# probabilists/azula

Hardware: AMD Instinct MI355X
Metric: images/sec (whole node), DDIM-64 256x256 UNet (higher is better)
Workload: dtype f32 (f16x2 split: 2 half pieces per operand, 3 partial products, f32 accumulate)

## Files before the change

### azula_amd/_lib.py

```python

from __future__ import annotations

import ctypes as C
import functools
import os
import threading

import torch

_HERE = os.path.dirname(os.path.abspath(__file__))
LIB_PATH = os.environ.get("AZULA_AMD_LIB") or os.path.join(_HERE, "csrc", "libazula_amd.so")

c_f32p = C.c_void_p
c_stream = C.c_void_p


class AzStepCoef(C.Structure):
    _fields_ = [
        ("c_in", C.c_float),
        ("c_skip", C.c_float),
        ("c_out", C.c_float),
        ("c_time", C.c_float),
        ("alpha_t", C.c_float),
        ("alpha_s", C.c_float),
# ... 279 lines not shown
        ("qk_heads", C.c_int32),
        ("qk_tokens", C.c_int32),
        ("qk_rmsnorm", C.c_int32),
        ("qk_eps", C.c_float),
        ("qk_reserved", C.c_int32),
        ("qk_q_weight", c_f32p),
        ("qk_k_weight", c_f32p),
        ("qk_rope_cos", c_f32p),
        ("qk_rope_sin", c_f32p),
        ("depth_wrap", C.c_int32),
        ("dst_dtype", C.c_int32),
        ("w_scale", C.c_float),
        ("reserved1", C.c_int32),
        ("in_absmax0", c_f32p),
        ("in_absmax1", c_f32p),
    ]


class AzAttnArgs(C.Structure):
    _fields_ = [
        ("q", c_f32p),
        ("k", c_f32p),
        ("v", c_f32p),
        ("out", c_f32p),
        ("batch", C.c_int32),
        ("heads", C.c_int32),
        ("tokens", C.c_int32),
        ("head_dim", C.c_int32),
        ("q_bstride", C.c_int64),
        ("q_tstride", C.c_int64),
# ... 125 lines not shown
    "az_conv2d_winograd_f32": [C.POINTER(AzConvArgs), c_stream],
    "az_conv2d_winograd_suggest_splitk": [i64, i32, i32, i32, i32],
    "az_winograd_pack_filter_f32": [vp, vp, i32, i32, i32, i32, i32, i32, c_stream],
    "az_conv2d_winograd_x3_f32": [C.POINTER(AzConvArgs), c_stream],
    "az_winograd_pack_filter_x3_f32": [vp, vp, i32, i32, i32, i32, i32, i32, c_stream],
    "az_winograd_x3_choose_block": [i32, i32, i32, i32, vp, vp, vp, vp],
    "az_winograd_x3_block_geometry": [i32, i32, i32, i32, i32, i32, i32, vp, vp],
    "az_winograd_x3_structured_mask": [C.POINTER(AzConvArgs), vp, vp],
    "az_conv2d_f16x2_f32": [C.POINTER(AzConvArgs), c_stream],
    "az_conv2d_winograd_f16x2_f32": [C.POINTER(AzConvArgs), c_stream],
    "az_pack_conv_weight_f16x2_f32": [vp, vp, i32, i32, i32, i32, i32, i32, i32, f32, c_stream],
    "az_winograd_pack_filter_f16x2_f32": [vp, vp, i32, i32, i32, i32, i32, i32, f32, c_stream],
    "az_f16x2_weight_scale": [f32, i32],
    "az_absmax_f32": [vp, vp, i64, c_stream],
    "az_absmax_from_moments_f32": [vp, vp, i64, c_stream],
    "az_conv2d_winograd4_f32": [C.POINTER(AzConvArgs), c_stream],
    "az_conv2d_winograd4_suggest_splitk": [i64, i32, i32, i32, i32],
    "az_winograd4_pack_filter_f32": [vp, vp, i32, i32, i32, i32, i32, i32, c_stream],
    "az_pack_conv_weight_f32": [vp, vp, i32, i32, i32, i32, i32, i32, i32, c_stream],
    "az_attention_f32": [C.POINTER(AzAttnArgs), c_stream],
    "az_attention_x3_f32": [C.POINTER(AzAttnArgs), c_stream],
    "az_attention_f16x2_f32": [C.POINTER(AzAttnArgs), c_stream],
    "az_attention_bf16_f32": [C.POINTER(AzAttnArgs), c_stream],
    "az_attention_f16_f32": [C.POINTER(AzAttnArgs), c_stream],
    "az_qk_prep_f32": [vp, vp, vp, vp, i64, i64, i32, i32, i64, i64, i64, i64, i64, i64, i32, i32, f32, vp, vp, c_stream],
    "az_qk_prep_w_f32": [vp, vp, vp, vp, i64, i64, i32, i32, i64, i64, i64, i64, i64, i64, i32, i32, f32, vp, vp, vp, vp, c_stream],
    "az_qk_prep_bwd_f32": [vp, vp, vp, vp, vp, vp, i64, i64, i32, i32, i64, i64, i64, i64, i64, i64, i64, i64, i64, i32, i32, f32, vp, vp,
                           c_stream],
    "az_qk_prep_bwd_w_f32": [vp, vp, vp, vp, vp, vp, i64, i64, i32, i32, i64, i64, i64, i64, i64, i64, i64, i64, i64, i32, i32, f32, vp,
                             vp, vp, vp, c_stream],
# ... 86 lines not shown
```

### azula_amd/csrc/conv.hip

```cpp
#include "conv_shared.h"
#include <cstdio>
#include <cstdlib>
#include <type_traits>

namespace {

constexpr int BM = 128;
constexpr int BN = 128;
constexpr int BK = 32;
constexpr int LDSS = 36;
constexpr int TILE_F = (BM + BN) * LDSS;

#include "igemm_kloop.inc"
struct ConvP {
  AzConvArgs a;
  int npix;
  int cin_s;
  int nkc0;
  int nkc1;
  int nk;
  int kps;
  int tiles_m;
  int tiles_n;
  int asm_loop;
// ... 1423 lines not shown
    }
    epilogue_store<IO>(a, n, co, v);
  }
}

template <int IO = 0>
__global__ __launch_bounds__(256) void conv_splitk_reduce_stats_kernel(ConvP p, int cpix) {
  __shared__ float sh[3 * 256];
  const AzConvArgs& a = p.a;
  const int Q = a.cout_s / 4;
  const int hw = a.hout * a.wout;
  const int b = blockIdx.y, chunk = blockIdx.x;
  const int tid = threadIdx.x;
  const int slots = Q >= 256 ? 1 : 256 / Q;
  const int p0 = chunk * cpix, p1 = min(hw, p0 + cpix);
  for (int q0 = 0; q0 < Q; q0 += 256) {
    const int q = q0 + (Q >= 256 ? tid : tid % Q);
    const int slot = Q >= 256 ? 0 : tid / Q;
    float cnt = 0.f, pivot = 0.f, s1 = 0.f, s2 = 0.f;
    if (q < Q && slot < slots) {
      for (int px = p0 + slot; px < p1; px += slots) {
        const int n = b * hw + px;
        float4 v = make_float4(0.f, 0.f, 0.f, 0.f);
#pragma unroll 4
        for (int z = 0; z < a.splitk; ++z) {
          const float4 w = ld4(a.workspace + ((int64_t)z * p.npix + n) * a.cout_s + q * 4);
          v.x += w.x;
          v.y += w.y;
          v.z += w.z;
          v.w += w.w;
// ... 26 lines not shown
          if (nb > 0.f) {
            const float nn = cnt + nb, d = mb - mean;
            mean = mean + d * (nb / nn);
            m2 = (m2 + vb) + d * d * (cnt * nb / nn);
            cnt = nn;
          }
        }
      }
    }
    if (slot == 0 && q < Q) {
      float* out = a.gn_quads + (((int64_t)b * a.gn_chunks + chunk) * Q + q) * 4;
      out[0] = cnt;
      out[1] = mean;
      out[2] = m2;
      out[3] = 0.f;
    }
  }
}

constexpr int WT = 64;
constexpr int WC = 64;
constexpr int WK = 8;
constexpr int WU_STAGE = 16 * WC * WK;
constexpr int WV_STAGE = 16 * WT * WK;
constexpr int W_STAGE = WU_STAGE + WV_STAGE;
constexpr int W_OT = 4 * WC + 4;
constexpr int W_LDS_BYTES = (2 * WT * W_OT + 3 * WT + 384) * 4;



__device__ __forceinline__ int wswz(int row, int half) { return row * WK + 4 * (half ^ ((row >> 3) & 1)); }
// ... 792 lines not shown
    const int grid = az_stream_grid((int64_t)cp.npix * (a.cout_s / 4), 256);
    if (io == 1) hipLaunchKernelGGL(conv_splitk_reduce_kernel<1>, dim3(grid), dim3(256), 0, st, cp);
    else if (io == 2) hipLaunchKernelGGL(conv_splitk_reduce_kernel<2>, dim3(grid), dim3(256), 0, st, cp);
    else hipLaunchKernelGGL(conv_splitk_reduce_kernel<0>, dim3(grid), dim3(256), 0, st, cp);
  }
  return az_launch_status();
}

static int conv2d_direct(const AzConvArgs* a, az_stream_t stream, int half );

int az_conv2d_f32(const AzConvArgs* a, az_stream_t stream) { return conv2d_direct(a, stream, 0); }

int az_conv2d_stem_f32(const AzConvArgs* a, az_stream_t stream) {
  AZ_REQUIRE(a && a->src0 && a->weight && a->dst, AZ_E_NULL);
  AZ_REQUIRE(a->ksize == 3 && a->stride == 1 && a->pad == 1 && !a->aniso && !a->src1 && a->c1s == 0 && a->up0 == 0 && !a->gate &&
                 !a->res && !a->dst_nchw && !a->in_affine && a->depth == 0 && a->splitk <= 1 && (a->act == 0 || a->act == 1),
             AZ_E_UNSUPPORTED);
  AZ_REQUIRE(a->c0s >= 1 && a->c0s <= 4 && a->cout_s > 0 && a->cout_s % 4 == 0 && a->batch > 0 && a->hin > 0 && a->win > 0 &&
                 a->hout == a->hin && a->wout == a->win && a->h0 == a->hin && a->w0 == a->win,
             AZ_E_SHAPE);
  AZ_REQUIRE((int64_t)a->batch * a->hin * a->win * a->cout_s < (1ll << 40), AZ_E_SHAPE);
  AZ_REQUIRE(AZ_ALIGNED16(a->weight) && AZ_ALIGNED16(a->bias) && AZ_ALIGNED16(a->dst) && AZ_ALIGNED16(a->gn_quads), AZ_E_ALIGN);
  const int tiles_h = (a->hin + ST_TH - 1) / ST_TH, tiles_w = (a->win + ST_TW - 1) / ST_TW;
  const int tiles_img = tiles_h * tiles_w;
  AZ_REQUIRE((int64_t)a->batch * tiles_img < (1ll << 31), AZ_E_SHAPE);
  if (a->gn_quads) AZ_REQUIRE(a->gn_chunks == tiles_img, AZ_E_SHAPE);
  ConvP p{};
  p.a = *a;
  const dim3 grid((unsigned)(a->batch * tiles_img));
  hipStream_t st = az_s(stream);
  switch (a->c0s) {
// ... 11 lines not shown
int az_conv2d_f16x2_f32(const AzConvArgs* a, az_stream_t stream) { return conv2d_direct(a, stream, 4); }

static bool conv_pow2(float v) {
  int e;
  return v > 0.f && v < 3.0e38f && frexpf(v, &e) == 0.5f;
}

static void launch_igemm_half(const ConvP& p, bool f16, bool srch, dim3 grid, hipStream_t st) {
  if (f16 && srch) hipLaunchKernelGGL((conv_igemm_half_kernel<true, true>), grid, dim3(256), 0, st, p);
  else if (f16) hipLaunchKernelGGL((conv_igemm_half_kernel<true, false>), grid, dim3(256), 0, st, p);
  else if (srch) hipLaunchKernelGGL((conv_igemm_half_kernel<false, true>), grid, dim3(256), 0, st, p);
  else hipLaunchKernelGGL((conv_igemm_half_kernel<false, false>), grid, dim3(256), 0, st, p);
}

static int conv2d_direct(const AzConvArgs* a, az_stream_t stream, int half) {
  AZ_REQUIRE(!a || !a->in_affine, AZ_E_UNSUPPORTED);
  if (a && a->depth != 0)
    AZ_REQUIRE(a->depth > 0 && a->batch % a->depth == 0 && a->depth_shift > -a->depth && a->depth_shift < a->depth &&
                   a->cout_s != 4 && (!a->gate || a->gate_bstride == 0) && (a->depth_wrap == 0 || a->depth_wrap == 1),
               AZ_E_UNSUPPORTED);
  AZ_REQUIRE(a && a->src0 && a->weight && a->dst, AZ_E_NULL);
  AZ_REQUIRE(a->batch > 0 && a->hin > 0 && a->win > 0 && a->hout > 0 && a->wout > 0, AZ_E_SHAPE);
  if (a->depth > 0) {
    const int64_t span = (int64_t)BN / ((int64_t)a->hout * a->wout) + 2 + a->depth;
    AZ_REQUIRE(span * a->h0 * a->w0 * a->c0s * 4 < (1ll << 31) && span * a->h1 * a->w1 * a->c1s * 4 < (1ll << 31), AZ_E_SHAPE);
  }
  AZ_REQUIRE(a->c0s > 0 && a->c0s % 4 == 0 && a->c1s % 4 == 0 && a->cout_s > 0 && a->cout_s % 4 == 0, AZ_E_SHAPE);
  AZ_REQUIRE((a->c1s == 0) == (a->src1 == nullptr), AZ_E_SHAPE);
  AZ_REQUIRE((a->src_dtype == 0 || a->src_dtype == 1) && (a->dst_dtype == 0 || a->dst_dtype == 1), AZ_E_SHAPE);
  AZ_REQUIRE((a->src_dtype == 0 && a->dst_dtype == 0) || half == 1 || half == 2, AZ_E_UNSUPPORTED);
  if (a->src_dtype) AZ_REQUIRE(a->c0s % 8 == 0 && a->c1s % 8 == 0, AZ_E_SHAPE);
// ... 316 lines not shown
      p.tblocks = a->batch * x3_rect_blocks_per_image(p.tiles_h, p.tiles_w, rw, rh);
      wino_order(p, 16);
    }
  }
  p.ups = x3_launch_mask(p.a);
  if (h2) AZ_REQUIRE(conv_pow2(a->w_scale), AZ_E_SHAPE);
  p.out_scale = h2 ? 1.f / a->w_scale : 1.f;
  if (h2) AZ_REQUIRE(AZ_ALIGNED16(a->in_absmax0) && AZ_ALIGNED16(a->in_absmax1) && (a->in_absmax0 || !a->in_absmax1), AZ_E_ALIGN);
  hipStream_t st = az_s(stream);
  int rc = azi_winograd_x3_launch(p, (unsigned)splitk, st, h2);
  if (rc != AZ_OK) return rc;
  if (splitk > 1) {
    ConvP cp;
    cp.a = p.a;
    cp.a.gn_quads = a->gn_quads;
    cp.npix = p.npix;
    rc = launch_splitk_reduce(cp, st);
  }
  return rc;
}

static void wino_order(WinoP& p, int wk) {
  int env_gt = 0, env_gc = 0;
  if (const char* e = az_ab_env("AZ_WINO_RECT")) sscanf(e, "%d,%d", &env_gt, &env_gc);
  int gt = env_gt > 0 ? env_gt : 8, gc = env_gt > 0 ? (env_gc > 0 ? env_gc : p.cblocks) : (wk == 16 ? 2 : 4);
  while (gc > 1 && p.cblocks % gc) gc >>= 1;
  if (env_gt <= 0) gt = 32 / gc;
  while (gt > 1 && p.tblocks % gt) gt >>= 1;
  if (p.cblocks % gc || p.tblocks % gt) gt = 1, gc = p.cblocks;
  p.gt = gt, p.gc = gc;
// ... 32 lines not shown
                 AZ_ALIGNED16(a->gate) && AZ_ALIGNED16(a->res) && AZ_ALIGNED16(a->workspace),
             AZ_E_ALIGN);
  if (!a->dst_nchw) AZ_REQUIRE(AZ_ALIGNED16(a->dst), AZ_E_ALIGN);
  if (a->dst_nchw) AZ_REQUIRE(a->dst_c > 0 && a->dst_c <= a->cout_s, AZ_E_SHAPE);
  if (a->gate) AZ_REQUIRE(a->gate_bstride % 4 == 0, AZ_E_ALIGN);
  if (a->res && a->res_up) AZ_REQUIRE(((a->hout + 1) >> 1) <= a->hres && ((a->wout + 1) >> 1) <= a->wres, AZ_E_SHAPE);
  AZ_REQUIRE(a->splitk >= 1 && (a->splitk == 1 || a->workspace), AZ_E_SHAPE);
  const int64_t npix64 = (int64_t)a->batch * a->hout * a->wout;
  AZ_REQUIRE(npix64 < (1ll << 31), AZ_E_SHAPE);
  if (a->gn_quads && a->splitk == 1) {
    const int64_t tiles_img = (int64_t)((a->hout + 1) / 2) * ((a->wout + 1) / 2);
    AZ_REQUIRE(!a->dst_nchw && a->cout_s % WC == 0 && tiles_img % WT == 0 && a->hout % 2 == 0 &&
                   a->wout % 2 == 0 && a->gn_chunks == tiles_img / WT,
               AZ_E_UNSUPPORTED);
  }

  p.a = *a;
  p.npix = (int)npix64;
  p.tiles_h = (a->hout + 1) / 2;
  p.tiles_w = (a->wout + 1) / 2;
  p.ntiles = a->batch * p.tiles_h * p.tiles_w;
  p.nkc0 = (a->c0s + wk - 1) / wk;
  p.nkc1 = (a->c1s + wk - 1) / wk;
  p.nk = p.nkc0 + p.nkc1;
  {
    const int64_t tiles_img = (int64_t)p.tiles_h * p.tiles_w;
    const int64_t span = (WT + tiles_img - 1) / tiles_img + 1;
    AZ_REQUIRE(span * a->h0 * a->w0 * a->c0s * 4 < (1ll << 31), AZ_E_SHAPE);
    AZ_REQUIRE(span * a->h1 * a->w1 * a->c1s * 4 < (1ll << 31), AZ_E_SHAPE);
  }
  splitk = a->splitk;
  if (splitk > p.nk) splitk = p.nk;
  p.kps = (p.nk + splitk - 1) / splitk;
  splitk = (p.nk + p.kps - 1) / p.kps;
  p.a.splitk = splitk;
  AZ_REQUIRE(!a->gn_quads || (a->splitk == 1) == (splitk == 1), AZ_E_UNSUPPORTED);
  if (splitk > 1) p.a.gn_quads = nullptr;
  p.cblocks = (a->cout_s + WC - 1) / WC;
  p.tblocks = (p.ntiles + WT - 1) / WT;
  p.rect_w = WT, p.rect_h = 1;
  p.ups = 0;
  wino_order(p, wk);
  AZ_REQUIRE((int64_t)p.nk * p.cblocks * ustage_bytes <= (1ll << 31), AZ_E_SHAPE);
  return AZ_OK;
}

int az_conv2d_winograd_suggest_splitk(int64_t batch, int32_t hout, int32_t wout, int32_t cout_s, int32_t cin_s) {
  const int64_t tiles = batch * ((hout + 1) / 2) * ((wout + 1) / 2);
  const int64_t blocks = ((tiles + WT - 1) / WT) * ((cout_s + WC - 1) / WC);
  const int64_t nk = (cin_s + WK - 1) / WK;
  int64_t want = (256 + blocks - 1) / blocks;
  int64_t maxs = nk / 8;
// ... 1 lines not shown
  if (want > maxs) want = maxs;
  if (want > 16) want = 16;
  if (blocks >= 192) want = 1;
  return (int)(want < 1 ? 1 : want);
}

int az_conv2d_winograd4_f32(const AzConvArgs* a, az_stream_t stream) {
  AZ_REQUIRE(a && a->src0 && a->weight && a->dst, AZ_E_NULL);
  AZ_REQUIRE(a->ksize == 3 && a->stride == 1 && a->pad == 1 && !a->aniso && a->src_dtype == 0 && a->dst_dtype == 0, AZ_E_UNSUPPORTED);
  AZ_REQUIRE(a->batch > 0 && a->hin > 0 && a->win > 0 && a->hout == a->hin && a->wout == a->win, AZ_E_SHAPE);
  AZ_REQUIRE(a->c0s > 0 && a->c0s % 4 == 0 && a->c1s % 4 == 0 && a->cout_s > 0 && a->cout_s % 4 == 0, AZ_E_SHAPE);
  AZ_REQUIRE((a->c1s == 0) == (a->src1 == nullptr), AZ_E_SHAPE);
  AZ_REQUIRE((a->act >= 0 && a->act <= 4) || a->act == 6, AZ_E_UNSUPPORTED);
  if (a->act == 6) AZ_REQUIRE(a->res && !a->gate && !a->dst_nchw && !a->gn_quads, AZ_E_UNSUPPORTED);
  if (a->act == 4) AZ_REQUIRE(!a->gate && !a->res && !a->dst_nchw && !a->gn_quads && a->cout_s % 8 == 0, AZ_E_UNSUPPORTED);
  AZ_REQUIRE(!a->in_affine && a->depth == 0, AZ_E_UNSUPPORTED);
  AZ_REQUIRE(!a->aniso || (a->up0_w >= 0 && a->up0_w <= 4 && a->up1_w >= 0 && a->up1_w <= 4), AZ_E_SHAPE);
  AZ_REQUIRE(a->up0 >= 0 && a->up0 <= 4 && ((a->hin + (1 << a->up0) - 1) >> a->up0) <= a->h0 &&
                 ((a->win + (1 << az_upw(a, a->up0, a->up0_w)) - 1) >> az_upw(a, a->up0, a->up0_w)) <= a->w0,
             AZ_E_SHAPE);
  if (a->src1)
    AZ_REQUIRE(a->up1 >= 0 && a->up1 <= 4 && ((a->hin + (1 << a->up1) - 1) >> a->up1) <= a->h1 &&
                 ((a->win + (1 << az_upw(a, a->up1, a->up1_w)) - 1) >> az_upw(a, a->up1, a->up1_w)) <= a->w1,
             AZ_E_SHAPE);
  AZ_REQUIRE(AZ_ALIGNED16(a->src0) && AZ_ALIGNED16(a->src1) && AZ_ALIGNED16(a->weight) && AZ_ALIGNED16(a->bias) &&
                 AZ_ALIGNED16(a->gate) && AZ_ALIGNED16(a->res) && AZ_ALIGNED16(a->workspace),
             AZ_E_ALIGN);
  if (!a->dst_nchw) AZ_REQUIRE(AZ_ALIGNED16(a->dst), AZ_E_ALIGN);
  if (a->dst_nchw) AZ_REQUIRE(a->dst_c > 0 && a->dst_c <= a->cout_s, AZ_E_SHAPE);
  if (a->gate) AZ_REQUIRE(a->gate_bstride % 4 == 0, AZ_E_ALIGN);
  if (a->res && a->res_up) AZ_REQUIRE(((a->hout + 1) >> 1) <= a->hres && ((a->wout + 1) >> 1) <= a->wres, AZ_E_SHAPE);
// ... 63 lines not shown
```

### azula_amd/csrc/conv_shared.h

```cpp
#pragma once

#include "common.h"

namespace {

typedef float f32x16 __attribute__((ext_vector_type(16)));

__device__ __forceinline__ float4 ld4(const float* p) { return *reinterpret_cast<const float4*>(p); }


typedef unsigned int u32x4 __attribute__((ext_vector_type(4)));

__device__ __forceinline__ float4 buf_ld4(__amdgpu_buffer_rsrc_t rsrc, unsigned voff, unsigned soff) {
  const u32x4 v = __builtin_amdgcn_raw_buffer_load_b128(rsrc, (int)voff, (int)soff, 0);
  return __builtin_bit_cast(float4, v);
}

typedef float f32x2 __attribute__((ext_vector_type(2)));
typedef unsigned int u32x2 __attribute__((ext_vector_type(2)));

__device__ __forceinline__ f32x2 buf_ld2(__amdgpu_buffer_rsrc_t rsrc, unsigned voff, unsigned soff) {
  const u32x2 v = __builtin_amdgcn_raw_buffer_load_b64(rsrc, (int)voff, (int)soff, 0);
  return __builtin_bit_cast(f32x2, v);
}
// ... 11 lines not shown

__device__ __forceinline__ int az_depth_plane(const AzConvArgs& a, int b, bool& ok) {
  ok = true;
  if (a.depth <= 0) return b;
  const int bd = b % a.depth;
  int sb = bd + a.depth_shift;
  if (a.depth_wrap) sb = sb < 0 ? sb + a.depth : (sb >= a.depth ? sb - a.depth : sb);
  else ok = (unsigned)sb < (unsigned)a.depth;
  return b - bd + sb;
}
__device__ __forceinline__ int az_depth_base(const AzConvArgs& a, int b_first) {
  if (a.depth <= 0) return b_first;
  if (a.depth_wrap) return b_first - b_first % a.depth;
  const int s = b_first + a.depth_shift;
  return s > 0 ? s : 0;
}

static inline int az_upw(const AzConvArgs* a, int up, int up_w) { return a->aniso ? up_w : up; }

__device__ __forceinline__ int64_t epilogue_res_index(const AzConvArgs& a, int n, int b) {
  const int rem = n - b * (a.hout * a.wout);
  if (a.res_up) {
    const int oh = rem / a.wout, ow = rem - oh * a.wout;
    return ((int64_t)b * a.hres + (oh >> 1)) * a.wres + (ow >> 1);
  }
  return a.res_bcast ? rem : n;
}

template <int IO = 0>
__device__ __forceinline__ void epilogue_fetch(const AzConvArgs& a, int n, int b, int co, float4& gate, float4& res) {
// ... 339 lines not shown
```

### azula_amd/csrc/norm.hip

```cpp
#include "common.h"

namespace {

struct Moments {
  float n, mean, m2;
};

__device__ __forceinline__ Moments combine(Moments a, Moments b) {
  if (b.n == 0.f) return a;
  if (a.n == 0.f) return b;
  Moments r;
  r.n = a.n + b.n;
  const float d = b.mean - a.mean;
  const float f = b.n / r.n;
  r.mean = a.mean + d * f;
  r.m2 = a.m2 + b.m2 + d * d * a.n * f;
  return r;
}

template <int IO = 0>
__global__ __launch_bounds__(256) void gn_stats_vec_kernel(float* __restrict__ partials,
                                                           const float* __restrict__ x,
                                                           const float* __restrict__ x1, int c0s, int64_t HW, int C,
                                                           int cs, int groups, int nchunks, int qs) {
// ... 537 lines not shown
}

__global__ __launch_bounds__(256) void absmax_moments_kernel(float* __restrict__ slots, const float4* __restrict__ partials, int64_t count) {
  __shared__ float sh[4];
  float m = 0.f;
  for (int64_t i = (int64_t)blockIdx.x * 256 + threadIdx.x; i < count; i += (int64_t)gridDim.x * 256) {
    const float4 q = partials[i];
    if (q.x > 0.f) m = fmaxf(m, fabsf(q.y) + sqrtf(fmaxf(q.z, 0.f)));
  }
  m = az_wave_max(m);
  if ((threadIdx.x & 63) == 0) sh[threadIdx.x >> 6] = m;
  __syncthreads();
  if (threadIdx.x == 0) slots[blockIdx.x] = fmaxf(fmaxf(sh[0], sh[1]), fmaxf(sh[2], sh[3]));
}

}

template <int IO>
static int affine_act_h16_launch(float* y, const float* x, const float* x1, int64_t c0s, const float* S, const float* T, int64_t B,
                                 int64_t H, int64_t W, int64_t cs, int32_t act, int32_t pool, hipStream_t st) {
  if (pool == 2) {
    AZ_REQUIRE(W % 2 == 0, AZ_E_SHAPE);
    const int grid = az_stream_grid(B * H * (W / 2) * (cs / 4), 256);
    if (act == 1) hipLaunchKernelGGL((affine_act_pool_kernel<1, 1, IO>), dim3(grid), dim3(256), 0, st, y, x, x1, (int)c0s, S, T, B, (int)H, (int)W, (int)cs);
    else hipLaunchKernelGGL((affine_act_pool_kernel<0, 1, IO>), dim3(grid), dim3(256), 0, st, y, x, x1, (int)c0s, S, T, B, (int)H, (int)W, (int)cs);
  } else if (pool) {
    AZ_REQUIRE(H % 2 == 0 && W % 2 == 0, AZ_E_SHAPE);
    const int grid = az_stream_grid(B * (H / 2) * (W / 2) * (cs / 4), 256);
    if (act == 1) hipLaunchKernelGGL((affine_act_pool_kernel<1, 2, IO>), dim3(grid), dim3(256), 0, st, y, x, x1, (int)c0s, S, T, B, (int)H, (int)W, (int)cs);
    else hipLaunchKernelGGL((affine_act_pool_kernel<0, 2, IO>), dim3(grid), dim3(256), 0, st, y, x, x1, (int)c0s, S, T, B, (int)H, (int)W, (int)cs);
// ... 18 lines not shown
extern "C" {

int az_absmax_f32(float* slots, const float* x, int64_t n, az_stream_t stream) {
  AZ_REQUIRE(slots && x, AZ_E_NULL);
  AZ_REQUIRE(n > 0, AZ_E_SHAPE);
  AZ_REQUIRE(AZ_ALIGNED16(x) && AZ_ALIGNED16(slots), AZ_E_ALIGN);
  hipLaunchKernelGGL(absmax_kernel, dim3(AZ_ABSMAX_SLOTS), dim3(256), 0, az_s(stream), slots, x, n / 4, n);
  return az_launch_status();
}

int az_absmax_from_moments_f32(float* slots, const float* partials, int64_t count, az_stream_t stream) {
  AZ_REQUIRE(slots && partials, AZ_E_NULL);
  AZ_REQUIRE(count > 0, AZ_E_SHAPE);
  AZ_REQUIRE(AZ_ALIGNED16(partials) && AZ_ALIGNED16(slots), AZ_E_ALIGN);
  hipLaunchKernelGGL(absmax_moments_kernel, dim3(AZ_ABSMAX_SLOTS), dim3(256), 0, az_s(stream), slots, reinterpret_cast<const float4*>(partials), count);
  return az_launch_status();
}

int az_groupnorm_stats_f32(float* partials, const float* x, const float* x1, int64_t c0s, int64_t B, int64_t HW,
                           int64_t C, int64_t cs, int32_t groups, int32_t nchunks, az_stream_t stream) {
  AZ_REQUIRE(partials && x, AZ_E_NULL);
  if (x1) AZ_REQUIRE(c0s > 0 && c0s < cs && c0s % 4 == 0 && C == cs && AZ_ALIGNED16(x1), AZ_E_SHAPE);
  AZ_REQUIRE(B > 0 && HW > 0 && C > 0 && cs >= C && cs % 4 == 0 && groups > 0 && C % groups == 0 && nchunks > 0,
             AZ_E_SHAPE);
  AZ_REQUIRE(AZ_ALIGNED16(x), AZ_E_ALIGN);
  const int Cg = (int)(C / groups);
  const int q = (int)(cs / 4);
  int qs = 0;
  if (Cg % 4 == 0 && C == cs) {
    for (int d = q < 256 ? q : 256; d >= Cg / 4 && qs == 0; --d)
// ... 153 lines not shown
```

### azula_amd/csrc/wino_x3.hip

```cpp
#include "conv_shared.h"

#include <cstdlib>
#include <type_traits>

namespace {

typedef __bf16 bf16x8 __attribute__((ext_vector_type(8)));
typedef _Float16 f16x8 __attribute__((ext_vector_type(8)));

constexpr int XT = 64;
constexpr int XC = 64;
constexpr int XK = 16;
constexpr int X_ROW = XK * 4;
constexpr int X_FREQ = XT * X_ROW;
constexpr int X_HALF = 8 * X_FREQ;
constexpr int X_STAGE = 2 * X_HALF;
constexpr int X_SLOTS = 768;
constexpr int X_SLOT = 64;
constexpr int X_DOFF1 = X_STAGE + X_SLOTS * X_SLOT;
constexpr int X_OT = 2 * XC + 4;
constexpr int X_EPI_BYTES = (4 * XT * X_OT + 3 * XT + 384) * 4;
constexpr int X_LDS_BYTES = X_DOFF1 + 512 * 32 > X_EPI_BYTES ? X_DOFF1 + 512 * 32 : X_EPI_BYTES;
static_assert(X_LDS_BYTES >= X_DOFF1 + 512 * 32 && X_LDS_BYTES >= 4 * 128 * 64 * 4, "the epilogue reuses the K loop's LDS");
constexpr int XU_STEP_BYTES = 16 * XC * XK * 3 * 2;
// ... 578 lines not shown
    for (int k = 0; k < 8; ++k) {
      wm[k] = sh[k * 16 + tid];
      w2[k] = sh[128 + k * 16 + tid];
    }
    float hn = 64.f;
#pragma unroll
    for (int o = 1; o < 8; o <<= 1, hn *= 2.f)
#pragma unroll
      for (int k = 0; k < 8; k += 2 * o) chan(wm[k], w2[k], wm[k + o], w2[k + o], hn);
    const int chunk = RECT ? rg.rb : (t0 - b_first * tiles_img) / XT;
    float* out = a.gn_quads + ((((int64_t)b_first * a.gn_chunks + chunk) * (a.cout_s / 4)) + (cb * (XC / 4) + tid)) * 4;
    out[0] = 1024.f;
    out[1] = wm[0];
    out[2] = w2[0];
    out[3] = 0.f;
  }
}

}

template <int AFF, bool TAIL, bool H2, bool RECT, bool UPS = false>
static int launch_x3(const WinoP& p, unsigned splitk, hipStream_t st) {
  static std::atomic<uint64_t> lds_set{0};
  hipError_t e = az_max_dynamic_lds((const void*)conv_winograd_x3_kernel<AFF, TAIL, H2, RECT, UPS>, X_LDS_BYTES, lds_set);
  if (e != hipSuccess) return (int)e;
  hipLaunchKernelGGL((conv_winograd_x3_kernel<AFF, TAIL, H2, RECT, UPS>), dim3((unsigned)((int64_t)p.cblocks * p.tblocks), splitk), dim3(512), X_LDS_BYTES,
                     st, p);
  return az_launch_status();
}

// ... 26 lines not shown
```

### azula_amd/engine.py

```python

from __future__ import annotations

import ctypes as C
import math
import os
from typing import NamedTuple

import torch

from . import _lib
from ._lib import AzConvArgs, AzNormFinalizeArgs, AzTransitionArgs


def pad4(c: int) -> int:
    return (c + 3) // 4 * 4


def pad8(c: int) -> int:
    return (c + 7) // 8 * 8


HALF_ACT = os.environ.get("AZ_HALF_ACT", "1") != "0"


# ... 70 lines not shown
            return lst.pop()
        t = torch.empty(numel, dtype=dtype, device=self.device)
        self.all.append(t)
        return t

    def release(self, t: torch.Tensor) -> None:
        self.free.setdefault((t.numel(), t.dtype), []).append(t)

    @property
    def bytes(self) -> int:
        return sum(t.numel() * t.element_size() for t in self.all)


class Act:

    __slots__ = ("buf", "B", "H", "W", "C", "cs", "pinned", "gn_quads", "affine", "qk_prepared", "bounded", "absmax")

    @property
    def half(self) -> bool:
        return self.buf.dtype != torch.float32

    def __init__(self, buf: torch.Tensor, B: int, H: int, W: int, C_: int, cs: int, pinned: bool = False) -> None:
        self.buf, self.B, self.H, self.W, self.C, self.cs, self.pinned = buf, B, H, W, C_, cs, pinned
        self.bounded = False
        self.absmax = None
        self.gn_quads = None
        self.qk_prepared = False
        self.affine = None

    @property
    def ptr(self) -> int:
        return self.buf.data_ptr()

    def view(self, B: int | None = None, H: int | None = None, W: int | None = None, C_: int | None = None, cs: int | None = None,
             *, buf: torch.Tensor | None = None, pinned: bool = True, bounded: bool | None = None, gn_quads: tuple | None = None) -> "Act":
        v = Act(self.buf if buf is None else buf, self.B if B is None else B, self.H if H is None else H, self.W if W is None else W,
                self.C if C_ is None else C_, self.cs if cs is None else cs, pinned)
        v.bounded = self.bounded if bounded is None else bounded
        v.gn_quads = gn_quads
        return v

# ... 1 lines not shown
WINOGRAD = os.environ.get("AZ_WINOGRAD", "1")
FP32_MFMA = os.environ.get("AZ_FP32_MFMA", "f16x2")
assert FP32_MFMA in ("native", "bf16x3", "f16x2"), FP32_MFMA


def moments_for_scale() -> bool:
    return FP32_MFMA == "f16x2" and F16X2_DYNAMIC and F16X2_MOMENTS


def pieces() -> bool:
    return FP32_MFMA in ("bf16x3", "f16x2")


F16X2_DYNAMIC = os.environ.get("AZ_F16X2_DYNAMIC", "1") != "0"
F16X2_MOMENTS = os.environ.get("AZ_F16X2_MOMENTS", "1") != "0"
ATTN_H2 = os.environ.get("AZ_ATTN_H2", "1") != "0"
ATTN_X3 = os.environ.get("AZ_ATTN_X3", "1") != "0"
WINO_X3 = os.environ.get("AZ_WINO_X3", "1") != "0"
X3_MIN_CHANNELS = 32
WINOGRAD4_MIN_TILES = int(os.environ.get("AZ_WINOGRAD4_MIN_TILES", "1024"))
QK_PREP = os.environ.get("AZ_QK_PREP", "1") != "0"
GN_FUSED = os.environ.get("AZ_GN_FUSED", "1") != "0"
STEM_PLANAR = os.environ.get("AZ_STEM_PLANAR", "1") != "0"
AFFINE_FUSED = os.environ.get("AZ_AFFINE_FUSED", "1") != "0"
GN_FUSED_SPLITK = os.environ.get("AZ_GN_FUSED", "1") != "epilogue"


WINO_X3_NAMES = ("az_conv2d_winograd_x3_f32", "az_conv2d_winograd_f16x2_f32")
H2_NAMES = ("az_conv2d_winograd_f16x2_f32", "az_conv2d_f16x2_f32")
PACKED = {"az_conv2d_winograd4_f32": "winograd4", "az_conv2d_winograd_f32": "winograd", "az_conv2d_winograd_x3_f32": "winograd_x3",
# ... 170 lines not shown
        n, args = self._wino_args(8, 1)
        return self._form("wino", n, torch.float32, "az_winograd_pack_filter_f32", *args)

    def winograd_x3(self) -> torch.Tensor:
        n, args = self._wino_args(16, 3)
        return self._form("wino_x3", n, torch.int16, "az_winograd_pack_filter_x3_f32", *args)

    def winograd4(self) -> torch.Tensor:
        nk, cb = (self.c0s + self.c1s) // 4, (self.cout_s + 63) // 64
        return self._form("wino4", nk * cb * 36 * 64 * 4, torch.float32, "az_winograd4_pack_filter_f32",
                          self.cout, self.cin, self.cin0, self.c0s, nk, cb)


class Builder:

    def __init__(self, device: torch.device, half: torch.dtype | None = None, half_act: bool = False) -> None:
        self.device = device
        self.half = half if half in (torch.bfloat16, torch.float16) else None
        self.half_act = bool(half_act) and self.half is not None and HALF_ACT
        self.tape = Tape()
        self.pool = Pool(device)
        self._ws_need = 0
        self._ws_users: list[AzConvArgs] = []
        self.workspace: torch.Tensor | None = None
        self._writes = 0
        self._last_write: dict[int, int] = {}

    def pad(self, c: int) -> int:
        return pad8(c) if self.half_act else pad4(c)

    def new_act(self, B: int, H: int, W: int, C_: int, pinned: bool = False, f32: bool = False) -> Act:
        cs = self.pad(C_)
        dtype = self.half if (self.half_act and not f32) else torch.float32
        return Act(self.pool.alloc(B * H * W * cs, dtype), B, H, W, C_, cs, pinned)

    def free(self, a: Act) -> None:
        if not a.pinned:
            self.pool.release(a.buf)

# ... 125 lines not shown
            else:
                tmp_src = self.materialize(src0)
                a.src0 = tmp_src.ptr
        moments = None
        if gn_stats and GN_FUSED and out is not None and cout == a.cout_s:
            if (name in ("az_conv2d_winograd_f32", *WINO_X3_NAMES) and a.splitk == 1 and cout % 64 == 0 and hout % 2 == 0
                    and wout % 2 == 0 and ((hout // 2) * (wout // 2)) % 64 == 0):
                moments = self._moments(a, B, cout, ((hout // 2) * (wout // 2)) // 64)
            elif GN_FUSED_SPLITK and a.splitk > 1 and name != "az_conv2d_winograd4_f32" and not (name == "az_conv2d_f32" and a.cout_s == 4):
                hw = hout * wout
                cpix = 2 * max(1, 256 // (cout // 4))
                chunks = max(1, min(128, (hw + cpix - 1) // cpix))
                while (hw + chunks - 1) // chunks * (chunks - 1) >= hw:
                    chunks -= 1
                moments = self._moments(a, B, cout, chunks)
        if (qk_prep is not None and QK_PREP and name in ("az_conv2d_f32", "az_conv2d_bf16_f32", "az_conv2d_f16_f32", "az_conv2d_x3_f32", "az_conv2d_f16x2_f32")
                and a.splitk == 1 and act == 0 and gate is None and res is None and out is not None and a.cout_s == cout
                and qk_prep["head_dim"] in (32, 64, 128) and cout == 3 * qk_prep["heads"] * qk_prep["head_dim"]):
            self._qk_prep(a, qk_prep, name, hout * wout)
        if a.splitk > 1:
            self._ws_need = max(self._ws_need, a.splitk * npix * a.cout_s)
            self._ws_users.append(a)
        a._flops = 2 * npix * cout * (src0.C + (src1.C if src1 is not None else 0)) * ks * ks
        a._algo = name
        self.tape.add(name, C.byref(a), keep=[a] if gate is None else [gate, a])
        if tmp_src is not None:
            self.free(tmp_src)
        if out is not None:
            self.wrote(out, bounded=False, moments=moments)
            out.qk_prepared = a.act == 5
        return out

    def _source(self, s: Act) -> ConvSource:
        return ConvSource(s.C, s.buf.numel(), s.bounded, s.affine is not None, self.fact(s, s.absmax) is not None,
                          self.fact(s, s.gn_quads) is not None)

    def _moments(self, a: AzConvArgs, B: int, cout: int, chunks: int) -> tuple:
        quads = self.empty(B * chunks * (cout // 4) * 4)
        a.gn_quads, a.gn_chunks = quads.data_ptr(), chunks
        return quads, chunks

    def _qk_prep(self, a: AzConvArgs, qk_prep: dict, name: str, tokens: int) -> None:
        a.act = 5
        if name != "az_conv2d_f32" and _lib.lib().az_conv2d_x3_suggest_splitk(C.byref(a)) != 1:
# ... 13 lines not shown
        a = AzConvArgs()
        a.src0, a.c0s, a.h0, a.w0 = x.data_ptr(), cin, H, W
        a.batch, a.hin, a.win, a.hout, a.wout = B, H, W, H, W
        a.weight = packed.stem().data_ptr()
        a.bias = packed.bias.data_ptr() if packed.bias is not None else None
        a.cout_s, a.ksize, a.stride, a.pad, a.splitk = cout, 3, 1, 1, 1
        a.pad_mode = 1 if periodic else 0
        out = self.new_act(B, H, W, cout)
        a.dst = out.ptr
        moments = self._moments(a, B, cout, ((H + 7) // 8) * ((W + 31) // 32)) if gn_stats and GN_FUSED else None
        a._flops = 0
        a._algo = "az_conv2d_stem_f32"
        self.tape.add("az_conv2d_stem_f32", C.byref(a), keep=[a, x])
        return self.wrote(out, bounded=False, moments=moments)

    def wrote(self, y: Act, *, bounded: bool, moments: tuple | None = None) -> Act:
        self._writes += 1
        self._last_write[y.buf.untyped_storage().data_ptr()] = self._writes
        y.bounded, y.absmax = bounded, None
        y.gn_quads = (*moments, self._writes) if moments is not None else None
        return y

    def fact(self, x: Act, rec: tuple | None) -> tuple | None:
        return rec if rec is not None and rec[-1] == self._last_write.get(x.buf.untyped_storage().data_ptr()) else None

    def absmax_of(self, x: Act) -> torch.Tensor:
        if self.fact(x, x.absmax) is None:
            assert not x.half and x.affine is None
            slots = self.empty(256)
            moments = self.fact(x, x.gn_quads)
            if moments is not None and F16X2_MOMENTS:
                self.tape.add("az_absmax_from_moments_f32", slots.data_ptr(), moments[0].data_ptr(), moments[0].numel() // 4, keep=[moments[0]])
            else:
                self.tape.add("az_absmax_f32", slots.data_ptr(), x.ptr, x.B * x.H * x.W * x.cs, keep=[x.buf])
            x.absmax = (slots, self._last_write.get(x.buf.untyped_storage().data_ptr()))
        return x.absmax[0]

    def upsample_nearest(self, x: Act, sh: int, sw: int, hout: int, wout: int) -> Act:
        y = self.new_act(x.B, hout, wout, x.C)
        self.tape.add("az_upsample_nearest_f32", y.ptr, x.ptr, x.B, x.H, x.W, x.cs, sh, sw, hout, wout)
        return self.wrote(y, bounded=False)

    def conv_dgrad(self, g: Act, conv, *, cin_lo: int = 0, cin_hi: int | None = None, res: Act | None = None,
                   dst_nchw: torch.Tensor | None = None, cache: dict | None = None, winograd=None) -> Act | None:
        w = conv.weight
        cin_hi = w.shape[1] if cin_hi is None else cin_hi
        key = (id(conv), cin_lo, cin_hi)
        packed = None if cache is None else cache.get(key)
# ... 540 lines not shown
```

### azula_amd/nn/unet.py

```python

from __future__ import annotations

from collections.abc import Sequence

import torch
import torch.nn as nn
from torch import Tensor

from ..engine import Act, Builder, Tape, ada_zero_triple, mod_front_tape, pad4
from .. import _lib, engine

__all__ = ["UNet", "UNetBlock"]


def _conv_holder(cin: int, cout: int, kernel_size, stride=1, identity_init: bool = False) -> nn.Module:
    Conv = {1: nn.Conv1d, 2: nn.Conv2d, 3: nn.Conv3d}[len(kernel_size)]
    conv = Conv(cin, cout, kernel_size=tuple(kernel_size), stride=stride, padding=tuple(k // 2 for k in kernel_size))
    if identity_init:
        center = [k // 2 for k in conv.weight.shape[2:]]
        eye = torch.zeros_like(conv.weight.data[:cin])
        for i in range(min(cin, cout)):
            eye[(i, i, *center)] = 1.0
        conv.weight.data[:cin].mul_(1e-2)
        conv.weight.data[:cin].add_(eye)
# ... 248 lines not shown
def _copy_tape(t):
    c = Tape()
    c.extend(t)
    return c


class UNetPlan:

    def __init__(self, net: "UNet", B: int, H: int, W: int, mod_rows: int, device: torch.device) -> None:
        self.B, self.H, self.W = B, H, W
        sv0 = (net.stride, net.stride) if isinstance(net.stride, int) else tuple(net.stride)
        blocks = [m for m in net.modules() if isinstance(m, UNetBlock)]
        half_act = (net.spatial == 2 and all(c % 8 == 0 for c in net.hid_channels) and all(v in (1, 2, 4, 8, 16) for v in sv0)
                    and all(b.norm_kind != "group" or (b.channels // b.groups) % 4 == 0 for b in blocks)
                    and all(b.ffn[0].out_channels % 8 == 0 and b.channels <= 4096 for b in blocks))
        bld = self.bld = Builder(device, half=next(net.parameters()).dtype, half_act=half_act)
        cin = net.in_channels + net.cond_channels
        D = net.mod_features
        first = net.descent[0][0]
        self.planar = (engine.STEM_PLANAR and net.spatial == 2 and cin <= 4 and tuple(first.weight.shape[2:]) == (3, 3)
                       and first.out_channels % 4 == 0 and bld.half is None)
        if self.planar:
            self.x_in = Act(torch.empty(B * cin * H * W, dtype=torch.float32, device=device), B, H, W, cin, 0, True)
        else:
            self.x_in = Act(torch.zeros(B * H * W * bld.pad(cin), dtype=torch.float32, device=device), B, H, W, cin, bld.pad(cin), True)
        self.mod = torch.empty(max(mod_rows, 1), max(D, 1), dtype=torch.float32, device=device)
        self.mod_rows = mod_rows
        self.out = torch.empty(B, net.out_channels, H, W, dtype=torch.float32, device=device)
        self.versions = net._param_versions()
        L = len(net.hid_blocks)
        stride = net.stride
# ... 416 lines not shown
```

### azula_amd/plugins/adm/unet.py

```python

from __future__ import annotations

import math

import torch
import torch.nn as nn
from torch import Tensor

from ... import _lib, engine
from ...engine import Act, Builder, pad8
from ...nn.unet import _GradTapes

__all__ = ["UNetModel"]


_CONV = {1: nn.Conv1d, 2: nn.Conv2d, 3: nn.Conv3d}


def _zero(m: nn.Module) -> nn.Module:
    for p in m.parameters():
        p.detach().zero_()
    return m


# ... 57 lines not shown
    freqs = torch.exp(-math.log(max_period) * torch.arange(0, half, dtype=torch.float32) / half)
    args = torch.arange(steps)[:, None].float() * freqs[None]
    emb = torch.cat([torch.cos(args), torch.sin(args)], dim=-1)
    if dim % 2:
        emb = torch.cat([emb, torch.zeros_like(emb[:, :1])], dim=-1)
    return emb


class ADMPlan:

    def __init__(self, net: "UNetModel", B: int, H: int, W: int, emb_rows: int, device, x_in: Act | None = None,
                 coef_ptr: int | None = None, frac: bool = False, D: int = 1) -> None:
        chans = sorted({m.num_channels for m in net.modules() if isinstance(m, nn.GroupNorm)})
        half_act = (net.dims != 3 and all(c % 128 == 0 for c in chans) and net.model_channels % 8 == 0
                    and (x_in is None or x_in.cs == pad8(net.in_channels)))
        bld = self.bld = Builder(device, half=next(net.parameters()).dtype, half_act=half_act)
        mc, E = net.model_channels, 4 * net.model_channels
        self.versions = net._param_versions()
        self.emb_rows = emb_rows
        cin = net.in_channels
        one_d = net.dims == 1
        assert not one_d or H == 1
        three_d = net.dims == 3
        assert three_d or D == 1
        PB = B * D
        up2 = (0, 1) if one_d else 1
        down2 = (1, 2) if one_d else 2
        pool2 = 2 if one_d else 1
        wino = False if one_d else None

        def packed(conv, **kw):
# ... 693 lines not shown
```

### include/azula_amd.h

```cpp
#ifndef AZULA_AMD_H
#define AZULA_AMD_H

#include <stdint.h>

#ifdef __cplusplus
extern "C" {
#endif

#define AZ_VERSION 1

enum {
  AZ_OK = 0,
  AZ_E_NULL = -1,
  AZ_E_SHAPE = -2,
  AZ_E_ALIGN = -3,
  AZ_E_UNSUPPORTED = -4
};

typedef void* az_stream_t;

int az_version(void);
const char* az_error_string(int code);

typedef struct AzStepCoef {
// ... 320 lines not shown
  int32_t qk_heads;
  int32_t qk_tokens;
  int32_t qk_rmsnorm;
  float qk_eps;
  int32_t qk_reserved;
  const float* qk_q_weight;
  const float* qk_k_weight;
  const float* qk_rope_cos;
  const float* qk_rope_sin;
  int32_t depth_wrap;
  int32_t dst_dtype;
  float w_scale;
  int32_t reserved1;
  const float* in_absmax0;
  const float* in_absmax1;
} AzConvArgs;
int az_conv2d_f32(const AzConvArgs* args, az_stream_t stream);
int az_conv2d_stem_f32(const AzConvArgs* args, az_stream_t stream);
int az_conv2d_bf16_f32(const AzConvArgs* args, az_stream_t stream);
int az_conv2d_f16_f32(const AzConvArgs* args, az_stream_t stream);
int az_conv2d_x3_f32(const AzConvArgs* args, az_stream_t stream);
int az_conv2d_x3_suggest_splitk(const AzConvArgs* args);
int az_conv2d_winograd_f32(const AzConvArgs* args, az_stream_t stream);
int az_conv2d_winograd_suggest_splitk(int64_t batch, int32_t hout, int32_t wout, int32_t cout_s, int32_t cin_s);
int az_conv2d_winograd_x3_f32(const AzConvArgs* args, az_stream_t stream);
int az_winograd_x3_choose_block(int32_t batch, int32_t hin, int32_t win, int32_t whole, int32_t* rect_w, int32_t* rect_h,
                                int64_t* slots, int64_t* slots_run);
int az_winograd_x3_block_geometry(int32_t batch, int32_t hin, int32_t win, int32_t pad_mode, int32_t rect_w, int32_t rect_h,
                                  int32_t block, int32_t* slot_pix, int32_t* tile_info);
int az_winograd_x3_structured_mask(const AzConvArgs* args, int32_t* mask, int32_t* launch_mask);
#define AZ_F16X2_IN_SCALE 0.0625f
int az_conv2d_f16x2_f32(const AzConvArgs* args, az_stream_t stream);
int az_conv2d_winograd_f16x2_f32(const AzConvArgs* args, az_stream_t stream);
float az_f16x2_weight_scale(float amax, int32_t winograd);
#define AZ_ABSMAX_SLOTS 256
int az_absmax_f32(float* slots, const float* x, int64_t n, az_stream_t stream);
int az_absmax_from_moments_f32(float* slots, const float* partials, int64_t count, az_stream_t stream);
int az_conv2d_winograd4_f32(const AzConvArgs* args, az_stream_t stream);
int az_conv2d_winograd4_suggest_splitk(int64_t batch, int32_t hout, int32_t wout, int32_t cout_s, int32_t cin_s);
int az_conv2d_suggest_splitk(int64_t npix, int32_t cout_s, int32_t cin_s, int32_t ksize);
int az_pack_conv_weight_f32(float* dst, const float* src, int32_t cout, int32_t cin, int32_t ks, int32_t cout_s,
                            int32_t cin0, int32_t c0s, int32_t cin_s, az_stream_t stream);

typedef struct AzAttnArgs {
  const float* q;
  const float* k;
  const float* v;
  float* out;
  int32_t batch, heads, tokens, head_dim;
  int64_t q_bstride, q_tstride, q_hstride;
  int64_t k_bstride, k_tstride, k_hstride;
  int64_t v_bstride, v_tstride, v_hstride;
// ... 129 lines not shown
```

Baseline: 4.710.

## Fuse absmax bound computation into conv GroupNorm-stats epilogues

Winograd-x3 and split-k reduce-with-stats kernels now compute an absmax upper bound (|mean| + sqrt(m2)) from their GroupNorm moment records. They write it into 256-slot atomicMax arrays taken from a preallocated arena, so the separate az_absmax_from_moments launches before f16x2 convolutions are no longer needed. One batched reset kernel per tape clears all arena slots. The aim is to cut kernel launches and an extra pass over the moment partials, at the cost of atomics and added epilogue work.

```diff
diff --git a/azula_amd/_lib.py b/azula_amd/_lib.py
--- a/azula_amd/_lib.py
+++ b/azula_amd/_lib.py
@@ -317,6 +317,7 @@
         ("reserved1", C.c_int32),
         ("in_absmax0", c_f32p),
         ("in_absmax1", c_f32p),
+        ("out_absmax", c_f32p),
     ]
 
 
@@ -472,6 +473,7 @@
     "az_f16x2_weight_scale": [f32, i32],
     "az_absmax_f32": [vp, vp, i64, c_stream],
     "az_absmax_from_moments_f32": [vp, vp, i64, c_stream],
+    "az_absmax_reset_f32": [vp, i64, c_stream],
     "az_conv2d_winograd4_f32": [C.POINTER(AzConvArgs), c_stream],
     "az_conv2d_winograd4_suggest_splitk": [i64, i32, i32, i32, i32],
     "az_winograd4_pack_filter_f32": [vp, vp, i32, i32, i32, i32, i32, i32, c_stream],
diff --git a/azula_amd/csrc/conv.hip b/azula_amd/csrc/conv.hip
--- a/azula_amd/csrc/conv.hip
+++ b/azula_amd/csrc/conv.hip
@@ -1461,6 +1461,7 @@
   const int tid = threadIdx.x;
   const int slots = Q >= 256 ? 1 : 256 / Q;
   const int p0 = chunk * cpix, p1 = min(hw, p0 + cpix);
+  float bm = 0.f;
   for (int q0 = 0; q0 < Q; q0 += 256) {
     const int q = q0 + (Q >= 256 ? tid : tid % Q);
     const int slot = Q >= 256 ? 0 : tid / Q;
@@ -1517,7 +1518,15 @@
       out[1] = mean;
       out[2] = m2;
       out[3] = 0.f;
-    }
+      bm = fmaxf(bm, az_record_bound(cnt, mean, m2));
+    }
+  }
+  if (a.out_absmax != nullptr) {
+    bm = az_wave_max(bm);
+    __syncthreads();
+    if ((tid & 63) == 0) sh[tid >> 6] = bm;
+    __syncthreads();
+    if (tid == 0) az_absmax_commit(a.out_absmax, fmaxf(fmaxf(sh[0], sh[1]), fmaxf(sh[2], sh[3])), blockIdx.y * gridDim.x + blockIdx.x);
   }
 }
 
@@ -2340,7 +2349,7 @@
 int az_conv2d_stem_f32(const AzConvArgs* a, az_stream_t stream) {
   AZ_REQUIRE(a && a->src0 && a->weight && a->dst, AZ_E_NULL);
   AZ_REQUIRE(a->ksize == 3 && a->stride == 1 && a->pad == 1 && !a->aniso && !a->src1 && a->c1s == 0 && a->up0 == 0 && !a->gate &&
-                 !a->res && !a->dst_nchw && !a->in_affine && a->depth == 0 && a->splitk <= 1 && (a->act == 0 || a->act == 1),
+                 !a->res && !a->dst_nchw && !a->in_affine && a->depth == 0 && a->splitk <= 1 && (a->act == 0 || a->act == 1) && !a->out_absmax,
              AZ_E_UNSUPPORTED);
   AZ_REQUIRE(a->c0s >= 1 && a->c0s <= 4 && a->cout_s > 0 && a->cout_s % 4 == 0 && a->batch > 0 && a->hin > 0 && a->win > 0 &&
                  a->hout == a->hin && a->wout == a->win && a->h0 == a->hin && a->w0 == a->win,
@@ -2382,7 +2391,7 @@
 }
 
 static int conv2d_direct(const AzConvArgs* a, az_stream_t stream, int half) {
-  AZ_REQUIRE(!a || !a->in_affine, AZ_E_UNSUPPORTED);
+  AZ_REQUIRE(!a || (!a->in_affine && !a->out_absmax), AZ_E_UNSUPPORTED);
   if (a && a->depth != 0)
     AZ_REQUIRE(a->depth > 0 && a->batch % a->depth == 0 && a->depth_shift > -a->depth && a->depth_shift < a->depth &&
                    a->cout_s != 4 && (!a->gate || a->gate_bstride == 0) && (a->depth_wrap == 0 || a->depth_wrap == 1),
@@ -2729,6 +2738,7 @@
     ConvP cp;
     cp.a = p.a;
     cp.a.gn_quads = a->gn_quads;
+    cp.a.out_absmax = a->gn_quads ? a->out_absmax : nullptr;
     cp.npix = p.npix;
     rc = launch_splitk_reduce(cp, st);
   }
@@ -2791,6 +2801,8 @@
                    a->wout % 2 == 0 && a->gn_chunks == tiles_img / WT,
                AZ_E_UNSUPPORTED);
   }
+  AZ_REQUIRE(!a->out_absmax || wk == 16, AZ_E_UNSUPPORTED);
+  AZ_REQUIRE(AZ_ALIGNED16(a->out_absmax), AZ_E_ALIGN);
 
   p.a = *a;
   p.npix = (int)npix64;
@@ -2812,7 +2824,7 @@
   splitk = (p.nk + p.kps - 1) / p.kps;
   p.a.splitk = splitk;
   AZ_REQUIRE(!a->gn_quads || (a->splitk == 1) == (splitk == 1), AZ_E_UNSUPPORTED);
-  if (splitk > 1) p.a.gn_quads = nullptr;
+  if (splitk > 1) p.a.gn_quads = nullptr, p.a.out_absmax = nullptr;
   p.cblocks = (a->cout_s + WC - 1) / WC;
   p.tblocks = (p.ntiles + WT - 1) / WT;
   p.rect_w = WT, p.rect_h = 1;
@@ -2844,7 +2856,7 @@
   AZ_REQUIRE((a->act >= 0 && a->act <= 4) || a->act == 6, AZ_E_UNSUPPORTED);
   if (a->act == 6) AZ_REQUIRE(a->res && !a->gate && !a->dst_nchw && !a->gn_quads, AZ_E_UNSUPPORTED);
   if (a->act == 4) AZ_REQUIRE(!a->gate && !a->res && !a->dst_nchw && !a->gn_quads && a->cout_s % 8 == 0, AZ_E_UNSUPPORTED);
-  AZ_REQUIRE(!a->in_affine && a->depth == 0, AZ_E_UNSUPPORTED);
+  AZ_REQUIRE(!a->in_affine && a->depth == 0 && !a->out_absmax, AZ_E_UNSUPPORTED);
   AZ_REQUIRE(!a->aniso || (a->up0_w >= 0 && a->up0_w <= 4 && a->up1_w >= 0 && a->up1_w <= 4), AZ_E_SHAPE);
   AZ_REQUIRE(a->up0 >= 0 && a->up0 <= 4 && ((a->hin + (1 << a->up0) - 1) >> a->up0) <= a->h0 &&
                  ((a->win + (1 << az_upw(a, a->up0, a->up0_w)) - 1) >> az_upw(a, a->up0, a->up0_w)) <= a->w0,
diff --git a/azula_amd/csrc/conv_shared.h b/azula_amd/csrc/conv_shared.h
--- a/azula_amd/csrc/conv_shared.h
+++ b/azula_amd/csrc/conv_shared.h
@@ -49,6 +49,13 @@
   if (a.depth_wrap) return b_first - b_first % a.depth;
   const int s = b_first + a.depth_shift;
   return s > 0 ? s : 0;
+}
+
+__device__ __forceinline__ float az_record_bound(float n, float mean, float m2) {
+  return n > 0.f ? fmaxf(0.f, fabsf(mean) + sqrtf(fmaxf(m2, 0.f))) : 0.f;
+}
+__device__ __forceinline__ void az_absmax_commit(float* slots, float m, unsigned wg) {
+  if (m > 0.f) atomicMax(reinterpret_cast<unsigned*>(slots) + (wg & (AZ_ABSMAX_SLOTS - 1)), __builtin_bit_cast(unsigned, m));
 }
 
 static inline int az_upw(const AzConvArgs* a, int up, int up_w) { return a->aniso ? up_w : up; }
diff --git a/azula_amd/csrc/norm.hip b/azula_amd/csrc/norm.hip
--- a/azula_amd/csrc/norm.hip
+++ b/azula_amd/csrc/norm.hip
@@ -575,6 +575,10 @@
   if (threadIdx.x == 0) slots[blockIdx.x] = fmaxf(fmaxf(sh[0], sh[1]), fmaxf(sh[2], sh[3]));
 }
 
+__global__ __launch_bounds__(256) void absmax_reset_kernel(float4* __restrict__ slots, int64_t n4) {
+  for (int64_t i = (int64_t)blockIdx.x * 256 + threadIdx.x; i < n4; i += (int64_t)gridDim.x * 256) slots[i] = make_float4(0.f, 0.f, 0.f, 0.f);
+}
+
 }
 
 template <int IO>
@@ -623,6 +627,14 @@
   AZ_REQUIRE(count > 0, AZ_E_SHAPE);
   AZ_REQUIRE(AZ_ALIGNED16(partials) && AZ_ALIGNED16(slots), AZ_E_ALIGN);
   hipLaunchKernelGGL(absmax_moments_kernel, dim3(AZ_ABSMAX_SLOTS), dim3(256), 0, az_s(stream), slots, reinterpret_cast<const float4*>(partials), count);
+  return az_launch_status();
+}
+
+int az_absmax_reset_f32(float* slots, int64_t n, az_stream_t stream) {
+  AZ_REQUIRE(slots, AZ_E_NULL);
+  AZ_REQUIRE(n > 0 && n % 4 == 0, AZ_E_SHAPE);
+  AZ_REQUIRE(AZ_ALIGNED16(slots), AZ_E_ALIGN);
+  hipLaunchKernelGGL(absmax_reset_kernel, dim3(az_stream_grid(n / 4, 256)), dim3(256), 0, az_s(stream), reinterpret_cast<float4*>(slots), n / 4);
   return az_launch_status();
 }
 
diff --git a/azula_amd/csrc/wino_x3.hip b/azula_amd/csrc/wino_x3.hip
--- a/azula_amd/csrc/wino_x3.hip
+++ b/azula_amd/csrc/wino_x3.hip
@@ -616,6 +616,12 @@
     out[1] = wm[0];
     out[2] = w2[0];
     out[3] = 0.f;
+    if (a.out_absmax != nullptr) {
+      float bm = az_record_bound(1024.f, wm[0], w2[0]);
+#pragma unroll
+      for (int o = 8; o > 0; o >>= 1) bm = fmaxf(bm, __shfl_xor(bm, o, 16));
+      if (tid == 0) az_absmax_commit(a.out_absmax, bm, blockIdx.x);
+    }
   }
 }
 
diff --git a/azula_amd/engine.py b/azula_amd/engine.py
--- a/azula_amd/engine.py
+++ b/azula_amd/engine.py
@@ -108,7 +108,7 @@
 
 class Act:
 
-    __slots__ = ("buf", "B", "H", "W", "C", "cs", "pinned", "gn_quads", "affine", "qk_prepared", "bounded", "absmax")
+    __slots__ = ("buf", "B", "H", "W", "C", "cs", "pinned", "gn_quads", "affine", "qk_prepared", "bounded", "absmax", "absmax_epi")
 
     @property
     def half(self) -> bool:
@@ -119,6 +119,7 @@
         self.bounded = False
         self.absmax = None
         self.gn_quads = None
+        self.absmax_epi = None
         self.qk_prepared = False
         self.affine = None
 
@@ -150,6 +151,8 @@
 
 F16X2_DYNAMIC = os.environ.get("AZ_F16X2_DYNAMIC", "1") != "0"
 F16X2_MOMENTS = os.environ.get("AZ_F16X2_MOMENTS", "1") != "0"
+ABSMAX_EPILOGUE = os.environ.get("AZ_ABSMAX_EPILOGUE", "1") != "0"
+ABSMAX_ARENA_SETS = 256
 ATTN_H2 = os.environ.get("AZ_ATTN_H2", "1") != "0"
 ATTN_X3 = os.environ.get("AZ_ATTN_X3", "1") != "0"
 WINO_X3 = os.environ.get("AZ_WINO_X3", "1") != "0"
@@ -350,8 +353,9 @@
 
 class Builder:
 
-    def __init__(self, device: torch.device, half: torch.dtype | None = None, half_act: bool = False) -> None:
+    def __init__(self, device: torch.device, half: torch.dtype | None = None, half_act: bool = False, absmax_epilogue: bool = False) -> None:
         self.device = device
+        self.absmax_epilogue = bool(absmax_epilogue)
         self.half = half if half in (torch.bfloat16, torch.float16) else None
         self.half_act = bool(half_act) and self.half is not None and HALF_ACT
         self.tape = Tape()
@@ -359,6 +363,9 @@
         self._ws_need = 0
         self._ws_users: list[AzConvArgs] = []
         self.workspace: torch.Tensor | None = None
+        self._slot_arena: torch.Tensor | None = None
+        self._slot_sets = 0
+        self._slot_reset: tuple | None = None
         self._writes = 0
         self._last_write: dict[int, int] = {}
 
@@ -514,6 +521,11 @@
                 while (hw + chunks - 1) // chunks * (chunks - 1) >= hw:
                     chunks -= 1
                 moments = self._moments(a, B, cout, chunks)
+        slots = None
+        if moments is not None and self.absmax_epilogue and ABSMAX_EPILOGUE and moments_for_scale() and name in WINO_X3_NAMES:
+            slots = self._absmax_slots()
+            if slots is not None:
+                a.out_absmax = slots.data_ptr()
         if (qk_prep is not None and QK_PREP and name in ("az_conv2d_f32", "az_conv2d_bf16_f32", "az_conv2d_f16_f32", "az_conv2d_x3_f32", "az_conv2d_f16x2_f32")
                 and a.splitk == 1 and act == 0 and gate is None and res is None and out is not None and a.cout_s == cout
                 and qk_prep["head_dim"] in (32, 64, 128) and cout == 3 * qk_prep["heads"] * qk_prep["head_dim"]):
@@ -527,7 +539,7 @@
         if tmp_src is not None:
             self.free(tmp_src)
         if out is not None:
-            self.wrote(out, bounded=False, moments=moments)
+            self.wrote(out, bounded=False, moments=moments, absmax=slots)
             out.qk_prepared = a.act == 5
         return out
 
@@ -571,11 +583,26 @@
         self.tape.add("az_conv2d_stem_f32", C.byref(a), keep=[a, x])
         return self.wrote(out, bounded=False, moments=moments)
 
-    def wrote(self, y: Act, *, bounded: bool, moments: tuple | None = None) -> Act:
+    def _absmax_slots(self) -> torch.Tensor | None:
+        if self._slot_sets == ABSMAX_ARENA_SETS:
+            return None
+        if self._slot_arena is None:
+            self._slot_arena = torch.zeros(ABSMAX_ARENA_SETS * 256, dtype=torch.float32, device=self.device)
+        at = self._slot_sets * 256
+        if self._slot_reset is None or self._slot_reset[0] is not self.tape:
+            count = C.c_int64(0)
+            self.tape.add("az_absmax_reset_f32", self._slot_arena.data_ptr() + 4 * at, count, keep=[self._slot_arena])
+            self._slot_reset = (self.tape, count)
+        self._slot_sets += 1
+        self._slot_reset[1].value += 256
+        return self._slot_arena[at : at + 256]
+
+    def wrote(self, y: Act, *, bounded: bool, moments: tuple | None = None, absmax: torch.Tensor | None = None) -> Act:
         self._writes += 1
         self._last_write[y.buf.untyped_storage().data_ptr()] = self._writes
         y.bounded, y.absmax = bounded, None
         y.gn_quads = (*moments, self._writes) if moments is not None else None
+        y.absmax_epi = (absmax, self._writes) if moments is not None and absmax is not None else None
         return y
 
     def fact(self, x: Act, rec: tuple | None) -> tuple | None:
@@ -584,11 +611,15 @@
     def absmax_of(self, x: Act) -> torch.Tensor:
         if self.fact(x, x.absmax) is None:
             assert not x.half and x.affine is None
-            slots = self.empty(256)
-            moments = self.fact(x, x.gn_quads)
-            if moments is not None and F16X2_MOMENTS:
+            moments = self.fact(x, x.gn_quads) if F16X2_MOMENTS else None
+            epi = self.fact(x, x.absmax_epi) if moments is not None else None
+            if epi is not None:
+                slots = epi[0]
+            elif moments is not None:
+                slots = self.empty(256)
                 self.tape.add("az_absmax_from_moments_f32", slots.data_ptr(), moments[0].data_ptr(), moments[0].numel() // 4, keep=[moments[0]])
             else:
+                slots = self.empty(256)
                 self.tape.add("az_absmax_f32", slots.data_ptr(), x.ptr, x.B * x.H * x.W * x.cs, keep=[x.buf])
             x.absmax = (slots, self._last_write.get(x.buf.untyped_storage().data_ptr()))
         return x.absmax[0]
diff --git a/azula_amd/nn/unet.py b/azula_amd/nn/unet.py
--- a/azula_amd/nn/unet.py
+++ b/azula_amd/nn/unet.py
@@ -286,7 +286,7 @@
         half_act = (net.spatial == 2 and all(c % 8 == 0 for c in net.hid_channels) and all(v in (1, 2, 4, 8, 16) for v in sv0)
                     and all(b.norm_kind != "group" or (b.channels // b.groups) % 4 == 0 for b in blocks)
                     and all(b.ffn[0].out_channels % 8 == 0 and b.channels <= 4096 for b in blocks))
-        bld = self.bld = Builder(device, half=next(net.parameters()).dtype, half_act=half_act)
+        bld = self.bld = Builder(device, half=next(net.parameters()).dtype, half_act=half_act, absmax_epilogue=True)
         cin = net.in_channels + net.cond_channels
         D = net.mod_features
         first = net.descent[0][0]
diff --git a/azula_amd/plugins/adm/unet.py b/azula_amd/plugins/adm/unet.py
--- a/azula_amd/plugins/adm/unet.py
+++ b/azula_amd/plugins/adm/unet.py
@@ -95,7 +95,7 @@
         chans = sorted({m.num_channels for m in net.modules() if isinstance(m, nn.GroupNorm)})
         half_act = (net.dims != 3 and all(c % 128 == 0 for c in chans) and net.model_channels % 8 == 0
                     and (x_in is None or x_in.cs == pad8(net.in_channels)))
-        bld = self.bld = Builder(device, half=next(net.parameters()).dtype, half_act=half_act)
+        bld = self.bld = Builder(device, half=next(net.parameters()).dtype, half_act=half_act, absmax_epilogue=True)
         mc, E = net.model_channels, 4 * net.model_channels
         self.versions = net._param_versions()
         self.emb_rows = emb_rows
diff --git a/include/azula_amd.h b/include/azula_amd.h
--- a/include/azula_amd.h
+++ b/include/azula_amd.h
@@ -358,6 +358,7 @@
   int32_t reserved1;
   const float* in_absmax0;
   const float* in_absmax1;
+  float* out_absmax;
 } AzConvArgs;
 int az_conv2d_f32(const AzConvArgs* args, az_stream_t stream);
 int az_conv2d_stem_f32(const AzConvArgs* args, az_stream_t stream);
@@ -380,6 +381,7 @@
 #define AZ_ABSMAX_SLOTS 256
 int az_absmax_f32(float* slots, const float* x, int64_t n, az_stream_t stream);
 int az_absmax_from_moments_f32(float* slots, const float* partials, int64_t count, az_stream_t stream);
+int az_absmax_reset_f32(float* slots, int64_t n, az_stream_t stream);
 int az_conv2d_winograd4_f32(const AzConvArgs* args, az_stream_t stream);
 int az_conv2d_winograd4_suggest_splitk(int64_t batch, int32_t hout, int32_t wout, int32_t cout_s, int32_t cin_s);
 int az_conv2d_suggest_splitk(int64_t npix, int32_t cout_s, int32_t cin_s, int32_t ksize);
```

Measured after the change: 4.666. No clear change (-0.9%).
